# hangxu0304/DeepReduce

Measured on NVIDIA H100. Metric: ResNet-50 images/sec (whole job, device-timed, max over ranks), higher is better.
Workload: dtype bf16

## Files before the change

deepreduce_b200/models/resnet.py:

```python
from __future__ import annotations

import torch.nn as nn
import torch.nn.functional as F

from .fused_bn import bn_add_relu, bn_bn_add_relu, bn_relu, bn_relu_maxpool


class _BasicCifar(nn.Module):
    def __init__(self, inp, out, stride):
        super().__init__()
        self.conv1 = nn.Conv2d(inp, out, 3, stride, 1, bias=False)
        self.bn1 = nn.BatchNorm2d(out)
        self.conv2 = nn.Conv2d(out, out, 3, 1, 1, bias=False)
        self.bn2 = nn.BatchNorm2d(out)
        self.pad = None
        if stride != 1 or inp != out:
            self.pad = (out - inp, stride)

    def forward(self, x):
        y = F.relu(self.bn1(self.conv1(x)))
        y = self.bn2(self.conv2(y))
        if self.pad is not None:
            extra, s = self.pad
            x = F.pad(x[:, :, ::s, ::s], (0, 0, 0, 0, extra // 2, extra - extra // 2))
        return F.relu(x + y)


class ResNetCifar(nn.Module):
    def __init__(self, n: int = 3, num_classes: int = 10):
        super().__init__()
        self.conv1 = nn.Conv2d(3, 16, 3, 1, 1, bias=False)
        self.bn1 = nn.BatchNorm2d(16)
        layers, inp = [], 16
        for out, stride in ((16, 1), (32, 2), (64, 2)):
            for i in range(n):
                layers.append(_BasicCifar(inp, out, stride if i == 0 else 1))
                inp = out
        self.layers = nn.Sequential(*layers)
        self.fc = nn.Linear(64, num_classes)

    def forward(self, x):
        x = F.relu(self.bn1(self.conv1(x)))
        x = self.layers(x)
        x = F.adaptive_avg_pool2d(x, 1).flatten(1)
        return self.fc(x)


def resnet20(num_classes: int = 10) -> ResNetCifar:
    return ResNetCifar(3, num_classes)


class _Bottleneck(nn.Module):
    expansion = 4

    def __init__(self, inp, width, stride, downsample):
        super().__init__()
        out = width * self.expansion
        self.conv1 = nn.Conv2d(inp, width, 1, bias=False)
        self.bn1 = nn.BatchNorm2d(width)
        self.conv2 = nn.Conv2d(width, width, 3, stride, 1, bias=False)
        self.bn2 = nn.BatchNorm2d(width)
        self.conv3 = nn.Conv2d(width, out, 1, bias=False)
        self.bn3 = nn.BatchNorm2d(out)
        self.downsample = None
        if downsample:
            self.downsample = nn.Sequential(nn.Conv2d(inp, out, 1, stride, bias=False), nn.BatchNorm2d(out))

    def forward(self, x, skip=None, fork=False):
        skip = x if skip is None else skip
        xd = None if self.downsample is None else self.downsample[0](skip)
        y = bn_relu(self.conv1(x), self.bn1)
        y = bn_relu(self.conv2(y), self.bn2)
        y = self.conv3(y)
        if xd is None:
            return bn_add_relu(y, self.bn3, skip, fork=fork)
        o = bn_bn_add_relu(y, self.bn3, xd, self.downsample[1])
        return (o, None) if fork else o


class ResNet(nn.Module):
    def __init__(self, blocks=(3, 4, 6, 3), num_classes: int = 1000):
        super().__init__()
        self.conv1 = nn.Conv2d(3, 64, 7, 2, 3, bias=False)
        self.bn1 = nn.BatchNorm2d(64)
        self.maxpool = nn.MaxPool2d(3, 2, 1)
        stages, inp = [], 64
        for i, (n, width) in enumerate(zip(blocks, (64, 128, 256, 512))):
            for j in range(n):
                stride = 2 if (j == 0 and i > 0) else 1
                stages.append(_Bottleneck(inp, width, stride, downsample=(j == 0)))
                inp = width * 4
        self.layers = nn.Sequential(*stages)
        self.fc = nn.Linear(inp, num_classes)
        for m in self.modules():
            if isinstance(m, nn.Conv2d):
                nn.init.kaiming_normal_(m.weight, mode="fan_out", nonlinearity="relu")

    def forward(self, x):
        x, skip = bn_relu_maxpool(self.conv1(x), self.bn1, self.maxpool), None
        for blk in self.layers:
            x, skip = blk(x, skip, fork=True)
        x = F.adaptive_avg_pool2d(x, 1).flatten(1)
        return self.fc(x)


def resnet50(num_classes: int = 1000) -> ResNet:
    return ResNet((3, 4, 6, 3), num_classes)
```

deepreduce_b200/ops/csrc/bn.cu:

```cuda
#include <cuda_bf16.h>

#include <algorithm>

#include "common.cuh"
#include "ops.h"

namespace dr {

namespace {

constexpr int kVec = 8;
constexpr int kApplyThreads = 256;
constexpr int kReduceThreads = 128;

struct ChanParams {
  float m[kVec], inv[kVec], w[kVec], b[kVec];
};

__device__ __forceinline__ void load8(const float* __restrict__ p, float* d) {
  const float4 a = __ldg(reinterpret_cast<const float4*>(p));
  const float4 b = __ldg(reinterpret_cast<const float4*>(p) + 1);
  d[0] = a.x; d[1] = a.y; d[2] = a.z; d[3] = a.w;
  d[4] = b.x; d[5] = b.y; d[6] = b.z; d[7] = b.w;
}

__device__ __forceinline__ void load_params(const BnParams& p, int c, ChanParams& o) {
  load8(p.mean + c, o.m);
  load8(p.invstd + c, o.inv);
  load8(p.weight + c, o.w);
  load8(p.bias + c, o.b);
}

__device__ __forceinline__ float bn_elem(float x, float m, float inv, float w, float b) {
  return __fmaf_rn(__fmul_rn(w, __fsub_rn(x, m)), inv, b);
}

__device__ __forceinline__ __nv_bfloat16 relu_bf16(__nv_bfloat16 v) {
  return __bfloat162float(v) <= 0.f ? __float2bfloat16_rn(0.f) : v;
}

__device__ __forceinline__ uint4 add_bf16x8(const uint4& a, const uint4& b) {
  uint4 s;
  const __nv_bfloat16* ha = reinterpret_cast<const __nv_bfloat16*>(&a);
  const __nv_bfloat16* hb = reinterpret_cast<const __nv_bfloat16*>(&b);
  __nv_bfloat16* hs = reinterpret_cast<__nv_bfloat16*>(&s);
#pragma unroll
  for (int i = 0; i < kVec; ++i) hs[i] = __float2bfloat16_rn(__fadd_rn(__bfloat162float(ha[i]), __bfloat162float(hb[i])));
  return s;
}

template <int kMode>
__global__ void __launch_bounds__(kApplyThreads) bn_apply_kernel(const __nv_bfloat16* __restrict__ x, BnParams px,
                                                                 const __nv_bfloat16* __restrict__ z, BnParams pz,
                                                                 __nv_bfloat16* __restrict__ out,
                                                                 uint8_t* __restrict__ mask, int64_t rows, int C) {
  const int groups = C / kVec;
  const int rows_per_cta = blockDim.x / groups;
  const int rsub = threadIdx.x / groups;
  if (rsub >= rows_per_cta) return;
  const int c = (threadIdx.x % groups) * kVec;
  ChanParams a;
  load_params(px, c, a);
  ChanParams d;
  if (kMode == 2) load_params(pz, c, d);
  const int64_t step = (int64_t)gridDim.x * rows_per_cta;
#pragma unroll 2
  for (int64_t r = (int64_t)blockIdx.x * rows_per_cta + rsub; r < rows; r += step) {
    const int64_t off = r * C + c;
    const uint4 vx = *reinterpret_cast<const uint4*>(x + off);
    uint4 vz = make_uint4(0, 0, 0, 0);
    if (kMode != 0) vz = *reinterpret_cast<const uint4*>(z + off);
    const __nv_bfloat16* hx = reinterpret_cast<const __nv_bfloat16*>(&vx);
    const __nv_bfloat16* hz = reinterpret_cast<const __nv_bfloat16*>(&vz);
    uint4 vo;
    __nv_bfloat16* ho = reinterpret_cast<__nv_bfloat16*>(&vo);
    unsigned bits = 0;
#pragma unroll
    for (int i = 0; i < kVec; ++i) {
      __nv_bfloat16 y = __float2bfloat16_rn(bn_elem(__bfloat162float(hx[i]), a.m[i], a.inv[i], a.w[i], a.b[i]));
      if (kMode != 0) {
        const __nv_bfloat16 s = kMode == 1 ? hz[i]
                                           : __float2bfloat16_rn(bn_elem(__bfloat162float(hz[i]), d.m[i], d.inv[i], d.w[i], d.b[i]));
        y = __float2bfloat16_rn(__fadd_rn(__bfloat162float(y), __bfloat162float(s)));
      }
      ho[i] = relu_bf16(y);
      bits |= (__bfloat162float(ho[i]) <= 0.f ? 0u : 1u) << i;
    }
    *reinterpret_cast<uint4*>(out + off) = vo;
    mask[r * groups + c / kVec] = (uint8_t)bits;
  }
}


__global__ void __launch_bounds__(kApplyThreads) bn_apply_pool_kernel(const __nv_bfloat16* __restrict__ x, BnParams px,
                                                                      __nv_bfloat16* __restrict__ out,
                                                                      uint8_t* __restrict__ codes, int64_t orows,
                                                                      PoolGeom pg, int C) {
  const int groups = C / kVec;
  const int rows_per_cta = blockDim.x / groups;
  const int rsub = threadIdx.x / groups;
  if (rsub >= rows_per_cta) return;
  const int c = (threadIdx.x % groups) * kVec;
  ChanParams a;
  load_params(px, c, a);
  const int64_t step = (int64_t)gridDim.x * rows_per_cta;
  for (int64_t r = (int64_t)blockIdx.x * rows_per_cta + rsub; r < orows; r += step) {
    const int ow = (int)(r % pg.Wo);
    const int64_t t = r / pg.Wo;
    const int oh = (int)(t % pg.Ho);
    const int64_t n = t / pg.Ho;
    const int h0 = 2 * oh - 1, w0 = 2 * ow - 1;
    uint4 v[9];
#pragma unroll
    for (int k = 0; k < 9; ++k) {
      const int ih = h0 + k / 3, iw = w0 + k % 3;
      v[k] = ih >= 0 && ih < pg.H && iw >= 0 && iw < pg.W
                 ? *reinterpret_cast<const uint4*>(x + ((n * pg.H + ih) * pg.W + iw) * C + c)
                 : uint4{};
    }
    __nv_bfloat16 best[kVec];
    unsigned slot[kVec];
#pragma unroll
    for (int i = 0; i < kVec; ++i) {
      best[i] = __float2bfloat16_rn(-INFINITY);
      slot[i] = 0;
    }
#pragma unroll
    for (int k = 0; k < 9; ++k) {
      const int ih = h0 + k / 3, iw = w0 + k % 3;
      if (ih < 0 || ih >= pg.H || iw < 0 || iw >= pg.W) continue;
      const __nv_bfloat16* hx = reinterpret_cast<const __nv_bfloat16*>(&v[k]);
#pragma unroll
      for (int i = 0; i < kVec; ++i) {
        const __nv_bfloat16 y = relu_bf16(__float2bfloat16_rn(bn_elem(__bfloat162float(hx[i]), a.m[i], a.inv[i], a.w[i], a.b[i])));
        const float fy = __bfloat162float(y);
        if (fy > __bfloat162float(best[i]) || isnan(fy)) {
          best[i] = y;
          slot[i] = k;
        }
      }
    }
    uint4 vo;
    __nv_bfloat16* ho = reinterpret_cast<__nv_bfloat16*>(&vo);
    uint2 vc;
    uint8_t* hc = reinterpret_cast<uint8_t*>(&vc);
#pragma unroll
    for (int i = 0; i < kVec; ++i) {
      ho[i] = best[i];
      hc[i] = (uint8_t)(slot[i] | (__bfloat162float(best[i]) <= 0.f ? 0u : 0x80u));
    }
    *reinterpret_cast<uint4*>(out + r * C + c) = vo;
    *reinterpret_cast<uint2*>(codes + r * C + c) = vc;
  }
}

struct PoolGather {
  uint4 g[4];
  uint2 code[4];
  int off;
  int nh, nw;
  int sh, sw;
};

__device__ __forceinline__ void pool_gather_codes(PoolGather& q, const uint8_t* __restrict__ codes, const PoolGeom& pg,
                                                  int row, int C, int c, bool valid) {
  const int w = row % pg.W, t = row / pg.W, h = t % pg.H, n = t / pg.H;
  const int ph = h >> 1, pw = w >> 1;
  q.nh = valid ? min((h + 1) / 2 + 1, pg.Ho) - ph : 0;
  q.nw = valid ? min((w + 1) / 2 + 1, pg.Wo) - pw : 0;
  q.sh = h - 2 * ph + 1;
  q.sw = w - 2 * pw + 1;
  q.off = ((n * pg.Ho + ph) * pg.Wo + pw) * C + c;
#pragma unroll
  for (int k = 0; k < 4; ++k) {
    const int a = k >> 1, b = k & 1;
    q.code[k] = a < q.nh && b < q.nw ? *reinterpret_cast<const uint2*>(codes + q.off + (a * pg.Wo + b) * C) : uint2{};
  }
}

template <bool kTwo>
__device__ __forceinline__ void pool_gather_grads(PoolGather& q, const __nv_bfloat16* __restrict__ gp,
                                                  const __nv_bfloat16* __restrict__ gp2, const PoolGeom& pg, int C) {
#pragma unroll
  for (int k = 0; k < 4; ++k) {
    const int a = k >> 1, b = k & 1;
    const bool in = a < q.nh && b < q.nw;
    const int off = q.off + (a * pg.Wo + b) * C;
    q.g[k] = in ? *reinterpret_cast<const uint4*>(gp + off) : uint4{};
    if (kTwo && in) q.g[k] = add_bf16x8(q.g[k], *reinterpret_cast<const uint4*>(gp2 + off));
  }
}

__device__ __forceinline__ void pool_gather_resolve(const PoolGather& q, uint4& g, unsigned& bits) {
  __nv_bfloat16* hg = reinterpret_cast<__nv_bfloat16*>(&g);
  const bool single = q.nh == 1 && q.nw == 1;
  bits = 0;
#pragma unroll
  for (int i = 0; i < kVec; ++i) {
    float s = 0.f;
    __nv_bfloat16 one = __float2bfloat16_rn(0.f);
    unsigned bit = 0;
#pragma unroll
    for (int k = 0; k < 4; ++k) {
      const int a = k >> 1, b = k & 1;
      const unsigned code = (reinterpret_cast<const uint8_t*>(&q.code[k]))[i];
      if (a < q.nh && b < q.nw && (int)(code & 0x7fu) == (q.sh - 2 * a) * 3 + (q.sw - 2 * b)) {
        const __nv_bfloat16 v = (reinterpret_cast<const __nv_bfloat16*>(&q.g[k]))[i];
        s = __fadd_rn(s, __bfloat162float(v));
        one = v;
        bit = code >> 7;
      }
    }
    hg[i] = single ? one : __float2bfloat16_rn(s);
    bits |= bit << i;
  }
}

template <bool kTwo>
__global__ void __launch_bounds__(kApplyThreads) bn_pool_grad_kernel(const __nv_bfloat16* __restrict__ gp,
                                                                     const __nv_bfloat16* __restrict__ gp2,
                                                                     const uint8_t* __restrict__ codes,
                                                                     __nv_bfloat16* __restrict__ g, PoolGeom pg,
                                                                     int64_t rows, int C) {
  const int groups = C / kVec;
  const int rows_per_cta = blockDim.x / groups;
  const int rsub = threadIdx.x / groups;
  if (rsub >= rows_per_cta) return;
  const int c = (threadIdx.x % groups) * kVec;
  const int64_t step = (int64_t)gridDim.x * rows_per_cta;
#pragma unroll 2
  for (int64_t r = (int64_t)blockIdx.x * rows_per_cta + rsub; r < rows; r += step) {
    PoolGather q;
    pool_gather_codes(q, codes, pg, (int)r, C, c, true);
    pool_gather_grads<kTwo>(q, gp, gp2, pg, C);
    uint4 v;
    unsigned bits;
    pool_gather_resolve(q, v, bits);
    __nv_bfloat16* hv = reinterpret_cast<__nv_bfloat16*>(&v);
#pragma unroll
    for (int i = 0; i < kVec; ++i)
      if (!((bits >> i) & 1u)) hv[i] = __float2bfloat16_rn(0.f);
    *reinterpret_cast<uint4*>(g + r * C + c) = v;
  }
}

struct RowTree {
  int block_y, grid_y;
  __host__ __device__ int S() const { return block_y * grid_y; }
  __host__ __device__ int loops(int rows) const { return 1 + (rows - 1) / (S() * kLoads); }
  static constexpr int kLoads = 4;
};

constexpr int kStatsThreads = 256;

__device__ __forceinline__ void welford_update(float x, float inv, float valid, float& mean, float& m2n) {
  const float d0 = __fsub_rn(x, mean);
  mean = __fmaf_rn(d0, inv, mean);
  const float d1 = __fsub_rn(x, mean);
  m2n = __fmaf_rn(__fmul_rn(d0, d1), valid, m2n);
}

template <int kN, bool kFuseNew>
__device__ __forceinline__ void welford_merge(int& n, float* mean, float* m2n, int n_new, const float* mean_new,
                                              const float* m2n_new) {
  const float fn = (float)n, fn_new = (float)n_new;
  const float factor = __frcp_rn((float)max(1, n + n_new));
#pragma unroll
  for (int i = 0; i < kN; ++i) {
    const float d = __fsub_rn(mean[i], mean_new[i]);
    const float s = kFuseNew ? __fmaf_rn(mean_new[i], fn_new, __fmul_rn(mean[i], fn))
                             : __fmaf_rn(mean[i], fn, __fmul_rn(mean_new[i], fn_new));
    mean[i] = __fmul_rn(s, factor);
    const float u = __fmul_rn(__fmul_rn(__fmul_rn(d, d), fn_new), fn);
    m2n[i] = __fadd_rn(m2n[i], __fmaf_rn(u, factor, m2n_new[i]));
  }
  n += n_new;
}

template <int kN>
struct WelfordSlots {
  float* mean; float* m2n; int* count;
  __device__ WelfordSlots(float* sh, int slots)
      : mean(sh), m2n(sh + slots * kN), count(reinterpret_cast<int*>(sh + 2 * slots * kN)) {}
  __device__ void put(int s, int n, const float* m, const float* q) const {
#pragma unroll
    for (int i = 0; i < kN; ++i) { mean[s * kN + i] = m[i]; m2n[s * kN + i] = q[i]; }
    count[s] = n;
  }
  template <bool kFuseNew>
  __device__ void merge_from(int s, int& n, float* m, float* q) const {
    float mn[kN], qn[kN];
#pragma unroll
    for (int i = 0; i < kN; ++i) { mn[i] = mean[s * kN + i]; qn[i] = m2n[s * kN + i]; }
    welford_merge<kN, kFuseNew>(n, m, q, count[s], mn, qn);
  }
  static size_t bytes(int slots) { return (size_t)slots * (2 * kN * sizeof(float) + sizeof(int)); }
};

template <int kN>
__device__ __forceinline__ void welford_tree_over_y(const WelfordSlots<kN>& sl, bool part, int y, int block_y, int base,
                                                    int stride, int& n, float* mean, float* m2n) {
  for (int off = block_y / 2; off > 0; off >>= 1) {
    if (part && y < 2 * off) sl.put(base + y * stride, n, mean, m2n);
    __syncthreads();
    if (part && y < off) sl.template merge_from<false>(base + (y + off) * stride, n, mean, m2n);
    __syncthreads();
  }
}

struct StatsOut {
  float* mean; float* invstd; float* running_mean; float* running_var;
  float* st_mean; float* st_m2n; int* st_count;
  float momentum, bessel, eps;
};

__device__ __forceinline__ void stats_store(const StatsOut& o, int c, int n, float mean, float m2n) {
  const float var = __fdiv_rn(m2n, (float)n);
  const float keep = __fsub_rn(1.f, o.momentum);
  o.mean[c] = mean;
  o.invstd[c] = rsqrtf(__fadd_rn(var, o.eps));
  o.running_mean[c] = __fmaf_rn(mean, o.momentum, __fmul_rn(o.running_mean[c], keep));
  o.running_var[c] = __fmaf_rn(__fmul_rn(var, o.bessel), o.momentum, __fmul_rn(o.running_var[c], keep));
}

__global__ void __launch_bounds__(kStatsThreads) bn_stats_kernel(const __nv_bfloat16* __restrict__ x, StatsOut o,
                                                                 RowTree t, int rows, int C) {
  constexpr int L = RowTree::kLoads;
  constexpr int kAhead = 4;
  extern __shared__ float sh[];
  const int gpc = blockDim.x / (L * t.block_y);
  const int g = threadIdx.x % gpc, j = (threadIdx.x / gpc) % L, y = threadIdx.x / (gpc * L);
  const int group = blockIdx.x * gpc + g;
  const bool live = group * kVec < C;
  const int c = live ? group * kVec : 0;
  const int S = t.S();
  const int n_loops = t.loops(rows);
  const int r0 = blockIdx.y * t.block_y + y + j * S;
  const int rstep = L * S;
  float mean[kVec], m2n[kVec];
#pragma unroll
  for (int i = 0; i < kVec; ++i) mean[i] = m2n[i] = 0.f;
  int n = 0;
  auto load = [&](uint4* b, int i0) {
#pragma unroll
    for (int u = 0; u < kAhead; ++u) {
      const int r = r0 + (i0 + u) * rstep;
      b[u] = live && i0 + u < n_loops && r < rows ? *reinterpret_cast<const uint4*>(x + (size_t)r * C + c) : uint4{};
    }
  };
  uint4 cur[kAhead];
  load(cur, 0);
  for (int i0 = 0; i0 < n_loops; i0 += kAhead) {
    uint4 nxt[kAhead];
    load(nxt, i0 + kAhead);
#pragma unroll
    for (int u = 0; u < kAhead; ++u) {
      const int i = i0 + u;
      if (i >= n_loops) break;
      const bool valid = r0 + i * rstep < rows;
      const float inv = valid ? __frcp_rn((float)(i + 1)) : 0.f;
      const float fv = valid ? 1.f : 0.f;
      n += valid;
      const __nv_bfloat16* hx = reinterpret_cast<const __nv_bfloat16*>(&cur[u]);
#pragma unroll
      for (int k = 0; k < kVec; ++k) welford_update(__bfloat162float(hx[k]), inv, fv, mean[k], m2n[k]);
    }
#pragma unroll
    for (int u = 0; u < kAhead; ++u) cur[u] = nxt[u];
  }
  const WelfordSlots<kVec> sl(sh, blockDim.x);
  sl.put(threadIdx.x, n, mean, m2n);
  __syncthreads();
  if (j == 0) {
#pragma unroll
    for (int a = 1; a < L; ++a) sl.merge_from<true>(threadIdx.x + a * gpc, n, mean, m2n);
  }
  __syncthreads();
  welford_tree_over_y<kVec>(sl, j == 0, y, t.block_y, g, gpc * L, n, mean, m2n);
  if (j != 0 || y != 0 || !live) return;
  if (t.grid_y == 1) {
#pragma unroll
    for (int i = 0; i < kVec; ++i) stats_store(o, c + i, n, mean[i], m2n[i]);
    return;
  }
#pragma unroll
  for (int i = 0; i < kVec; ++i) {
    o.st_mean[(size_t)blockIdx.y * C + c + i] = mean[i];
    o.st_m2n[(size_t)blockIdx.y * C + c + i] = m2n[i];
  }
  if (group == 0) o.st_count[blockIdx.y] = n;
}

__global__ void bn_stats_finalize_kernel(StatsOut o, RowTree t, int C) {
  extern __shared__ float sh[];
  const int cols = blockDim.x / t.block_y;
  const int col = threadIdx.x % cols, y = threadIdx.x / cols;
  const int c = blockIdx.x * cols + col;
  int n = 0;
  float mean = 0.f, m2n = 0.f;
  if (c < C)
    for (int b = y; b < t.grid_y; b += t.block_y) {
      const float mb = o.st_mean[(size_t)b * C + c], qb = o.st_m2n[(size_t)b * C + c];
      welford_merge<1, false>(n, &mean, &m2n, o.st_count[b], &mb, &qb);
    }
  const WelfordSlots<1> sl(sh, blockDim.x);
  welford_tree_over_y<1>(sl, true, y, t.block_y, col, cols, n, &mean, &m2n);
  if (y == 0 && c < C) stats_store(o, c, n, mean, m2n);
}


template <int kN>
__device__ __forceinline__ void tree_over_y(float* v, float* sh, int y, int n, int col, int width) {
  for (int off = n / 2; off > 0; off >>= 1) {
#pragma unroll
    for (int i = 0; i < kN; ++i) sh[y * width + col + i] = v[i];
    __syncthreads();
    if (y < off) {
#pragma unroll
      for (int i = 0; i < kN; ++i) v[i] = __fadd_rn(v[i], sh[(y + off) * width + col + i]);
    }
    __syncthreads();
  }
}

struct BwdOut {
  float* sums;
  float* dw; float* db; float* dwz; float* dbz;
  float* staging;
};

__device__ __forceinline__ void bwd_store(const BwdOut& o, int k, int c, int C, float v, const float* invstd,
                                         const float* invstd_z) {
  o.sums[k * C + c] = v;
  if (k == 0) {
    o.db[c] = v;
    if (o.dbz) o.dbz[c] = v;
  } else if (k == 1) {
    o.dw[c] = __fmul_rn(v, invstd[c]);
  } else {
    o.dwz[c] = __fmul_rn(v, invstd_z[c]);
  }
}

__device__ __forceinline__ float masked(__nv_bfloat16 go, unsigned bit) { return bit ? __bfloat162float(go) : 0.f; }

template <int kMode, bool kTwo>
__global__ void __launch_bounds__(kReduceThreads) bn_bwd_reduce_kernel(const __nv_bfloat16* __restrict__ go,
                                                                       const __nv_bfloat16* __restrict__ go2,
                                                                       const uint8_t* __restrict__ mask,
                                                                       const __nv_bfloat16* __restrict__ x,
                                                                       const float* __restrict__ mean,
                                                                       const float* __restrict__ invstd,
                                                                       const __nv_bfloat16* __restrict__ z,
                                                                       const float* __restrict__ mean_z,
                                                                       const float* __restrict__ invstd_z,
                                                                       __nv_bfloat16* __restrict__ g_out, BwdOut o,
                                                                       RowTree t, int rows, int C) {
  constexpr int kSums = kMode == 2 ? 3 : 2;
  constexpr int L = RowTree::kLoads;
  extern __shared__ float sh[];
  const int gpc = blockDim.x / t.block_y;
  const int tg = threadIdx.x % gpc, y = threadIdx.x / gpc;
  const int group = blockIdx.x * gpc + tg;
  const bool live = group * kVec < C;
  const int c = live ? group * kVec : 0;
  const int S = t.S();
  float m[kVec], mz[kVec];
#pragma unroll
  for (int i = 0; i < kVec; ++i) {
    m[i] = mean[c + i];
    mz[i] = kMode == 2 ? mean_z[c + i] : 0.f;
  }
  float acc[kSums][L][kVec];
#pragma unroll
  for (int k = 0; k < kSums; ++k)
#pragma unroll
    for (int j = 0; j < L; ++j)
#pragma unroll
      for (int i = 0; i < kVec; ++i) acc[k][j][i] = 0.f;
  const int mgroups = C / kVec;
  int r = blockIdx.y * t.block_y + y;
  const int n_loops = t.loops(rows);
  constexpr bool kAhead = !(kTwo && kMode == 2);
  struct Batch {
    uint4 g[L], g2[L], x[L], z[L];
    unsigned m[L];
  };
  auto load = [&](Batch& b, int r0) {
#pragma unroll
    for (int j = 0; j < L; ++j) {
      const int rr = r0 + j * S;
      if (live && rr < rows) {
        const int off = rr * C + c;
        b.g[j] = *reinterpret_cast<const uint4*>(go + off);
        if (kTwo) b.g2[j] = *reinterpret_cast<const uint4*>(go2 + off);
        b.x[j] = *reinterpret_cast<const uint4*>(x + off);
        if (kMode == 2) b.z[j] = *reinterpret_cast<const uint4*>(z + off);
        b.m[j] = kMode == 3 ? 0u : mask[rr * mgroups + group];
      } else {
        b.g[j] = uint4{}; b.g2[j] = uint4{}; b.x[j] = uint4{}; b.z[j] = uint4{}; b.m[j] = 0;
      }
    }
  };
  Batch cur;
  if (kAhead) load(cur, r);
  for (int it = 0; it < n_loops; ++it) {
    if (!kAhead) load(cur, r);
    if (kTwo) {
#pragma unroll
      for (int j = 0; j < L; ++j) cur.g[j] = add_bf16x8(cur.g[j], cur.g2[j]);
    }
    Batch nxt;
    if (kAhead) load(nxt, r + L * S);
    const unsigned* mb = cur.m;
#pragma unroll
    for (int j = 0; j < L; ++j) {
      const __nv_bfloat16* hg = reinterpret_cast<const __nv_bfloat16*>(&cur.g[j]);
      const __nv_bfloat16* hx = reinterpret_cast<const __nv_bfloat16*>(&cur.x[j]);
      const __nv_bfloat16* hz = reinterpret_cast<const __nv_bfloat16*>(&cur.z[j]);
      uint4 vo;
      __nv_bfloat16* ho = reinterpret_cast<__nv_bfloat16*>(&vo);
#pragma unroll
      for (int i = 0; i < kVec; ++i) {
        const unsigned bit = (mb[j] >> i) & 1u;
        const float g = kMode == 3 ? __bfloat162float(hg[i]) : masked(hg[i], bit);
        if (kMode == 1) ho[i] = bit ? hg[i] : __float2bfloat16_rn(0.f);
        acc[0][j][i] = __fadd_rn(acc[0][j][i], g);
        acc[1][j][i] = __fmaf_rn(__fsub_rn(__bfloat162float(hx[i]), m[i]), g, acc[1][j][i]);
        if (kMode == 2) acc[2][j][i] = __fmaf_rn(__fsub_rn(__bfloat162float(hz[i]), mz[i]), g, acc[2][j][i]);
      }
      if (kMode == 1 && live && r + j * S < rows) *reinterpret_cast<uint4*>(g_out + (r + j * S) * C + c) = vo;
    }
    if (kAhead) cur = nxt;
    r += L * S;
  }
#pragma unroll
  for (int k = 0; k < kSums; ++k) {
#pragma unroll
    for (int i = 0; i < kVec; ++i)
#pragma unroll
      for (int j = 1; j < L; ++j) acc[k][0][i] = __fadd_rn(acc[k][0][i], acc[k][j][i]);
    tree_over_y<kVec>(acc[k][0], sh, y, t.block_y, tg * kVec, gpc * kVec);
  }
  if (y != 0 || !live) return;
#pragma unroll
  for (int k = 0; k < kSums; ++k)
#pragma unroll
    for (int i = 0; i < kVec; ++i) {
      if (t.grid_y > 1) o.staging[((size_t)k * t.grid_y + blockIdx.y) * C + c + i] = acc[k][0][i];
      else bwd_store(o, k, c + i, C, acc[k][0][i], invstd, invstd_z);
    }
}

__global__ void bn_bwd_finalize_kernel(BwdOut o, RowTree t, int n_sums, int C, const float* __restrict__ invstd,
                                       const float* __restrict__ invstd_z) {
  extern __shared__ float sh[];
  const int cols = blockDim.x / t.block_y;
  const int col = threadIdx.x % cols, y = threadIdx.x / cols;
  const int c = blockIdx.x * cols + col;
  for (int k = 0; k < n_sums; ++k) {
    float v = 0.f;
    if (c < C)
      for (int b = y; b < t.grid_y; b += t.block_y) v = __fadd_rn(v, o.staging[((size_t)k * t.grid_y + b) * C + c]);
    tree_over_y<1>(&v, sh, y, t.block_y, col, cols);
    if (y == 0 && c < C) bwd_store(o, k, c, C, v, invstd, invstd_z);
  }
}

struct ElemtChan {
  float m[kVec], f1[kVec], f2[kVec], sdy[kVec];
};

__device__ __forceinline__ void elemt_params(const float* mean, const float* invstd, const float* w, const float* sdy,
                                             const float* sxmu, float norm, int c, ElemtChan& p) {
  float inv[kVec], ww[kVec], sx[kVec];
  load8(mean + c, p.m);
  load8(invstd + c, inv);
  load8(w + c, ww);
  load8(sdy + c, p.sdy);
  load8(sxmu + c, sx);
#pragma unroll
  for (int i = 0; i < kVec; ++i) {
    p.f1[i] = __fmul_rn(__fmul_rn(__fmul_rn(inv[i], inv[i]), sx[i]), norm);
    p.f2[i] = __fmul_rn(ww[i], inv[i]);
  }
}

__device__ __forceinline__ __nv_bfloat16 elemt(float g, float x, const ElemtChan& p, int i, float norm) {
  const float a = __fmaf_rn(-p.sdy[i], norm, g);
  return __float2bfloat16_rn(__fmul_rn(__fmaf_rn(-p.f1[i], __fsub_rn(x, p.m[i]), a), p.f2[i]));
}

struct ElemtArgs {
  const float *mean, *invstd, *weight, *sums;
  const float *mean_z, *invstd_z, *weight_z;
};

template <int kMode, bool kTwo>
__global__ void __launch_bounds__(kApplyThreads) bn_bwd_elemt_kernel(const __nv_bfloat16* __restrict__ g_in,
                                                                     const __nv_bfloat16* __restrict__ g2_in,
                                                                     const uint8_t* __restrict__ mask,
                                                                     const __nv_bfloat16* __restrict__ x,
                                                                     const __nv_bfloat16* __restrict__ z, ElemtArgs a,
                                                                     __nv_bfloat16* __restrict__ dx,
                                                                     __nv_bfloat16* __restrict__ dz, float norm,
                                                                     int64_t rows, int C) {
  const int groups = C / kVec;
  const int rows_per_cta = blockDim.x / groups;
  const int rsub = threadIdx.x / groups;
  if (rsub >= rows_per_cta) return;
  const int c = (threadIdx.x % groups) * kVec;
  ElemtChan p;
  elemt_params(a.mean, a.invstd, a.weight, a.sums, a.sums + C, norm, c, p);
  ElemtChan q;
  if (kMode == 2) elemt_params(a.mean_z, a.invstd_z, a.weight_z, a.sums, a.sums + 2 * C, norm, c, q);
  const int64_t step = (int64_t)gridDim.x * rows_per_cta;
#pragma unroll 2
  for (int64_t r = (int64_t)blockIdx.x * rows_per_cta + rsub; r < rows; r += step) {
    const int64_t off = r * C + c;
    uint4 vg = *reinterpret_cast<const uint4*>(g_in + off);
    if (kTwo) vg = add_bf16x8(vg, *reinterpret_cast<const uint4*>(g2_in + off));
    const unsigned mb = kMode == 1 || kMode == 3 ? 0xffu : mask[r * groups + c / kVec];
    const uint4 vx = *reinterpret_cast<const uint4*>(x + off);
    uint4 vz = make_uint4(0, 0, 0, 0);
    if (kMode == 2) vz = *reinterpret_cast<const uint4*>(z + off);
    const __nv_bfloat16* hg = reinterpret_cast<const __nv_bfloat16*>(&vg);
    const __nv_bfloat16* hx = reinterpret_cast<const __nv_bfloat16*>(&vx);
    const __nv_bfloat16* hz = reinterpret_cast<const __nv_bfloat16*>(&vz);
    uint4 vo, vd;
    __nv_bfloat16* ho = reinterpret_cast<__nv_bfloat16*>(&vo);
    __nv_bfloat16* hd = reinterpret_cast<__nv_bfloat16*>(&vd);
#pragma unroll
    for (int i = 0; i < kVec; ++i) {
      const float g = masked(hg[i], (mb >> i) & 1u);
      ho[i] = elemt(g, __bfloat162float(hx[i]), p, i, norm);
      if (kMode == 2) hd[i] = elemt(g, __bfloat162float(hz[i]), q, i, norm);
    }
    *reinterpret_cast<uint4*>(dx + off) = vo;
    if (kMode == 2) *reinterpret_cast<uint4*>(dz + off) = vd;
  }
}

__global__ void bn_update_stats_kernel(const float* __restrict__ mean, float* __restrict__ var_invstd,
                                       float* __restrict__ running_mean, float* __restrict__ running_var, int C,
                                       float momentum, float bessel, float eps) {
  const int c = blockIdx.x * blockDim.x + threadIdx.x;
  if (c >= C) return;
  const float m = mean[c], v = var_invstd[c];
  const float unbiased_var = v * bessel;
  running_mean[c] = m * momentum + (1 - momentum) * running_mean[c];
  running_var[c] = unbiased_var * momentum + (1 - momentum) * running_var[c];
  var_invstd[c] = rsqrtf(v + eps);
}

template <typename K>
cudaError_t rows_grid(K kernel, int64_t rows, int C, int& grid, int& threads) {
  const int groups = C / kVec;
  const int rows_per_cta = groups >= kApplyThreads ? 1 : kApplyThreads / groups;
  threads = groups * rows_per_cta;
  int per_sm = 0;
  cudaError_t e = cudaOccupancyMaxActiveBlocksPerMultiprocessor(&per_sm, kernel, threads, 0);
  if (e != cudaSuccess) return e;
  int64_t g = (rows + rows_per_cta - 1) / rows_per_cta;
  const int64_t cap = (int64_t)(per_sm > 0 ? per_sm : 1) * sm_count();
  grid = (int)(g > cap ? cap : g);
  return cudaSuccess;
}

template <int kMode>
cudaError_t launch_apply(const void* x, const BnParams& px, const void* z, const BnParams& pz, void* out, void* mask,
                         int64_t rows, int C, cudaStream_t st) {
  if (rows == 0) return cudaSuccess;
  int grid = 0, threads = 0;
  cudaError_t e = rows_grid(bn_apply_kernel<kMode>, rows, C, grid, threads);
  if (e != cudaSuccess) return e;
  count_launch();
  bn_apply_kernel<kMode><<<grid, threads, 0, st>>>(reinterpret_cast<const __nv_bfloat16*>(x), px,
                                                   reinterpret_cast<const __nv_bfloat16*>(z), pz,
                                                   reinterpret_cast<__nv_bfloat16*>(out),
                                                   reinterpret_cast<uint8_t*>(mask), rows, C);
  return cudaGetLastError();
}

int last_pow2(unsigned n) {
  n |= n >> 1; n |= n >> 2; n |= n >> 4; n |= n >> 8; n |= n >> 16;
  return std::max<int>(1, (int)(n - (n >> 1)));
}

RowTree row_tree(int rows, int C) {
  const int block_x = std::min(last_pow2((unsigned)C), 32);
  const int block_y = std::min(last_pow2((unsigned)((rows + 15) / 16)), 512 / block_x);
  int grid_y = std::min((rows + block_y * 16 - 1) / (block_y * 16), 128);
  if (grid_y < 8) grid_y = 1;
  return {block_y, grid_y};
}

template <int kMode, bool kTwo>
cudaError_t launch_bwd_reduce(const BnBwd& b, const RowTree& t, const BwdOut& o, int rows, int C, cudaStream_t st) {
  const int groups = C / kVec;
  const int gpc = std::min(groups, std::max(1, kReduceThreads / t.block_y));
  const dim3 grid((groups + gpc - 1) / gpc, t.grid_y);
  const int threads = gpc * t.block_y;
  count_launch();
  bn_bwd_reduce_kernel<kMode, kTwo><<<grid, threads, threads * kVec * sizeof(float), st>>>(
      reinterpret_cast<const __nv_bfloat16*>(b.go), reinterpret_cast<const __nv_bfloat16*>(b.go2), b.mask,
      reinterpret_cast<const __nv_bfloat16*>(b.x), b.px.mean, b.px.invstd, reinterpret_cast<const __nv_bfloat16*>(b.z),
      b.pz.mean, b.pz.invstd, reinterpret_cast<__nv_bfloat16*>(b.g), o, t, rows, C);
  return cudaGetLastError();
}

template <int kMode, bool kTwo>
cudaError_t launch_bwd_elemt(const BnBwd& b, const ElemtArgs& a, int64_t rows, int C, cudaStream_t st) {
  int grid = 0, threads = 0;
  cudaError_t e = rows_grid(bn_bwd_elemt_kernel<kMode, kTwo>, rows, C, grid, threads);
  if (e != cudaSuccess) return e;
  const float norm = (float)(1.0 / (double)rows);
  count_launch();
  bn_bwd_elemt_kernel<kMode, kTwo><<<grid, threads, 0, st>>>(
      reinterpret_cast<const __nv_bfloat16*>(kMode == 1 || kMode == 3 ? b.g : b.go),
      reinterpret_cast<const __nv_bfloat16*>(b.go2), b.mask, reinterpret_cast<const __nv_bfloat16*>(b.x),
      reinterpret_cast<const __nv_bfloat16*>(b.z), a, reinterpret_cast<__nv_bfloat16*>(b.dx),
      reinterpret_cast<__nv_bfloat16*>(b.dz), norm, rows, C);
  return cudaGetLastError();
}

template <int kMode, bool kTwo>
cudaError_t launch_backward(const BnBwd& b, int64_t rows64, int C, cudaStream_t st) {
  const int rows = (int)rows64;
  const RowTree t = row_tree(rows, C);
  const BwdOut o{b.sums, b.dw, b.db, b.dwz, b.dbz, b.staging};
  cudaError_t e;
  if (kMode == 3) {
    int grid = 0, threads = 0;
    e = rows_grid(bn_pool_grad_kernel<kTwo>, rows64, C, grid, threads);
    if (e != cudaSuccess) return e;
    count_launch();
    bn_pool_grad_kernel<kTwo><<<grid, threads, 0, st>>>(reinterpret_cast<const __nv_bfloat16*>(b.go),
                                                        reinterpret_cast<const __nv_bfloat16*>(b.go2), b.mask,
                                                        reinterpret_cast<__nv_bfloat16*>(b.g), b.pool, rows64, C);
    e = cudaGetLastError();
    if (e != cudaSuccess) return e;
  }
  BnBwd bb = b;
  if (kMode == 3) bb.go = b.g;
  e = launch_bwd_reduce<kMode, kTwo && kMode != 3>(bb, t, o, rows, C, st);
  if (e != cudaSuccess) return e;
  if (t.grid_y > 1) {
    const int cols = std::max(1, 512 / t.block_y);
    const int threads = cols * t.block_y;
    count_launch();
    bn_bwd_finalize_kernel<<<(C + cols - 1) / cols, threads, threads * sizeof(float), st>>>(
        o, t, kMode == 2 ? 3 : 2, C, b.px.invstd, b.pz.invstd);
    e = cudaGetLastError();
    if (e != cudaSuccess) return e;
  }
  const ElemtArgs a{b.px.mean, b.px.invstd, b.px.weight, b.sums, b.pz.mean, b.pz.invstd, b.pz.weight};
  return launch_bwd_elemt<kMode, kTwo && kMode == 2>(b, a, rows64, C, st);
}

cudaError_t launch_stats(const BnStats& s, int rows, int C, cudaStream_t st) {
  const RowTree t = row_tree(rows, C);
  const int grid_y = t.grid_y;
  const StatsOut o{s.mean, s.invstd, s.running_mean, s.running_var,
                   s.staging, s.staging + (size_t)grid_y * C, reinterpret_cast<int*>(s.staging + 2 * (size_t)grid_y * C),
                   s.momentum, s.bessel, s.eps};
  const int groups = C / kVec;
  const int gpc = std::min(groups, std::max(1, kStatsThreads / (RowTree::kLoads * t.block_y)));
  const int threads = gpc * RowTree::kLoads * t.block_y;
  count_launch();
  bn_stats_kernel<<<dim3((groups + gpc - 1) / gpc, grid_y), threads, WelfordSlots<kVec>::bytes(threads), st>>>(
      reinterpret_cast<const __nv_bfloat16*>(s.x), o, t, rows, C);
  cudaError_t e = cudaGetLastError();
  if (e != cudaSuccess || grid_y == 1) return e;
  const int cols = std::max(1, 512 / t.block_y);
  const int fthreads = cols * t.block_y;
  count_launch();
  bn_stats_finalize_kernel<<<(C + cols - 1) / cols, fthreads, WelfordSlots<1>::bytes(fthreads), st>>>(o, t, C);
  return cudaGetLastError();
}

}

void bn_row_tree(int64_t rows, int C, int* block_y, int* grid_y) {
  const RowTree t = row_tree((int)rows, C);
  *block_y = t.block_y;
  *grid_y = t.grid_y;
}

cudaError_t launch_bn_backward(int mode, const BnBwd& b, int64_t rows, int C, cudaStream_t st) {
  if (rows == 0) return cudaSuccess;
  const bool two = b.go2 != nullptr;
  switch (mode) {
    case 0: return two ? cudaErrorInvalidValue : launch_backward<0, false>(b, rows, C, st);
    case 1: return two ? launch_backward<1, true>(b, rows, C, st) : launch_backward<1, false>(b, rows, C, st);
    case 2: return two ? launch_backward<2, true>(b, rows, C, st) : launch_backward<2, false>(b, rows, C, st);
    case 3: return two ? launch_backward<3, true>(b, rows, C, st) : launch_backward<3, false>(b, rows, C, st);
    default: return cudaErrorInvalidValue;
  }
}

cudaError_t launch_bn_stats(const BnStats& s, int64_t rows, int C, cudaStream_t st) {
  if (rows == 0) return cudaSuccess;
  return launch_stats(s, (int)rows, C, st);
}

cudaError_t launch_bn_update_stats(const float* mean, float* var_invstd, float* running_mean, float* running_var, int C,
                                   float momentum, float bessel, float eps, cudaStream_t st) {
  count_launch();
  bn_update_stats_kernel<<<(C + 255) / 256, 256, 0, st>>>(mean, var_invstd, running_mean, running_var, C, momentum,
                                                          bessel, eps);
  return cudaGetLastError();
}

cudaError_t launch_bn_apply(int mode, const void* x, const BnParams& px, const void* z, const BnParams& pz, void* out,
                            void* mask, int64_t rows, int C, cudaStream_t st) {
  switch (mode) {
    case 0: return launch_apply<0>(x, px, z, pz, out, mask, rows, C, st);
    case 1: return launch_apply<1>(x, px, z, pz, out, mask, rows, C, st);
    case 2: return launch_apply<2>(x, px, z, pz, out, mask, rows, C, st);
    default: return cudaErrorInvalidValue;
  }
}

cudaError_t launch_bn_apply_pool(const void* x, const BnParams& px, void* out, void* codes, int N, const PoolGeom& pg,
                                 int C, cudaStream_t st) {
  const int64_t orows = (int64_t)N * pg.Ho * pg.Wo;
  if (orows == 0) return cudaSuccess;
  int grid = 0, threads = 0;
  cudaError_t e = rows_grid(bn_apply_pool_kernel, orows, C, grid, threads);
  if (e != cudaSuccess) return e;
  count_launch();
  bn_apply_pool_kernel<<<grid, threads, 0, st>>>(reinterpret_cast<const __nv_bfloat16*>(x), px,
                                                 reinterpret_cast<__nv_bfloat16*>(out),
                                                 reinterpret_cast<uint8_t*>(codes), orows, pg, C);
  return cudaGetLastError();
}

}
```

Measured before the change: 6158.

## Tile fused BN-ReLU-maxpool forward and backward with shared-memory row reuse

Rewrites the stem BN+ReLU+maxpool forward kernel as a 2D-tiled kernel. A cp.async ring buffer stages input rows in shared memory, so each input pixel is normalized once and shared across overlapping 3x3 windows instead of being reloaded up to nine times. The pool-grad backward kernel is tiled the same way, walking output rows in bands and sharing neighbour gradients and codes through shared memory instead of gathering four per input pixel. The model also passes fork=True to the stem call, which changes the Python API expectation. It adds shared-memory use and __syncthreads, and relies on bn_relu_maxpool accepting the fork argument, which is not shown.

```diff
diff --git a/deepreduce_b200/models/resnet.py b/deepreduce_b200/models/resnet.py
--- a/deepreduce_b200/models/resnet.py
+++ b/deepreduce_b200/models/resnet.py
@@ -97,7 +97,7 @@
                 nn.init.kaiming_normal_(m.weight, mode="fan_out", nonlinearity="relu")
 
     def forward(self, x):
-        x, skip = bn_relu_maxpool(self.conv1(x), self.bn1, self.maxpool), None
+        x, skip = bn_relu_maxpool(self.conv1(x), self.bn1, self.maxpool, fork=True)
         for blk in self.layers:
             x, skip = blk(x, skip, fork=True)
         x = F.adaptive_avg_pool2d(x, 1).flatten(1)
diff --git a/deepreduce_b200/ops/csrc/bn.cu b/deepreduce_b200/ops/csrc/bn.cu
--- a/deepreduce_b200/ops/csrc/bn.cu
+++ b/deepreduce_b200/ops/csrc/bn.cu
@@ -91,105 +91,164 @@
   }
 }
 
-
-__global__ void __launch_bounds__(kApplyThreads) bn_apply_pool_kernel(const __nv_bfloat16* __restrict__ x, BnParams px,
-                                                                      __nv_bfloat16* __restrict__ out,
-                                                                      uint8_t* __restrict__ codes, int64_t orows,
-                                                                      PoolGeom pg, int C) {
-  const int groups = C / kVec;
-  const int rows_per_cta = blockDim.x / groups;
-  const int rsub = threadIdx.x / groups;
-  if (rsub >= rows_per_cta) return;
-  const int c = (threadIdx.x % groups) * kVec;
-  ChanParams a;
-  load_params(px, c, a);
-  const int64_t step = (int64_t)gridDim.x * rows_per_cta;
-  for (int64_t r = (int64_t)blockIdx.x * rows_per_cta + rsub; r < orows; r += step) {
-    const int ow = (int)(r % pg.Wo);
-    const int64_t t = r / pg.Wo;
-    const int oh = (int)(t % pg.Ho);
-    const int64_t n = t / pg.Ho;
-    const int h0 = 2 * oh - 1, w0 = 2 * ow - 1;
-    uint4 v[9];
-#pragma unroll
-    for (int k = 0; k < 9; ++k) {
-      const int ih = h0 + k / 3, iw = w0 + k % 3;
-      v[k] = ih >= 0 && ih < pg.H && iw >= 0 && iw < pg.W
-                 ? *reinterpret_cast<const uint4*>(x + ((n * pg.H + ih) * pg.W + iw) * C + c)
-                 : uint4{};
-    }
-    __nv_bfloat16 best[kVec];
-    unsigned slot[kVec];
-#pragma unroll
-    for (int i = 0; i < kVec; ++i) {
-      best[i] = __float2bfloat16_rn(-INFINITY);
-      slot[i] = 0;
-    }
-#pragma unroll
-    for (int k = 0; k < 9; ++k) {
-      const int ih = h0 + k / 3, iw = w0 + k % 3;
-      if (ih < 0 || ih >= pg.H || iw < 0 || iw >= pg.W) continue;
-      const __nv_bfloat16* hx = reinterpret_cast<const __nv_bfloat16*>(&v[k]);
-#pragma unroll
-      for (int i = 0; i < kVec; ++i) {
-        const __nv_bfloat16 y = relu_bf16(__float2bfloat16_rn(bn_elem(__bfloat162float(hx[i]), a.m[i], a.inv[i], a.w[i], a.b[i])));
-        const float fy = __bfloat162float(y);
-        if (fy > __bfloat162float(best[i]) || isnan(fy)) {
-          best[i] = y;
-          slot[i] = k;
-        }
-      }
-    }
-    uint4 vo;
-    __nv_bfloat16* ho = reinterpret_cast<__nv_bfloat16*>(&vo);
-    uint2 vc;
-    uint8_t* hc = reinterpret_cast<uint8_t*>(&vc);
-#pragma unroll
-    for (int i = 0; i < kVec; ++i) {
-      ho[i] = best[i];
-      hc[i] = (uint8_t)(slot[i] | (__bfloat162float(best[i]) <= 0.f ? 0u : 0x80u));
-    }
-    *reinterpret_cast<uint4*>(out + r * C + c) = vo;
-    *reinterpret_cast<uint2*>(codes + r * C + c) = vc;
-  }
+constexpr int kPoolThreads = 256;
+constexpr int kPoolSliceGroups = 32;
+constexpr int kPoolBand = 8;
+
+struct PoolTile {
+  int gs, slices;
+  int tile, tiles;
+  int band, bands;
+  int threads;
+  int64_t ctas;
+};
+
+struct PoolCta {
+  int64_t n;
+  int oh0, oh1;
+  int ow0;
+  int owl, gl, c;
+  bool group;
+};
+
+__device__ __forceinline__ PoolCta pool_cta(const PoolTile& t, const PoolGeom& pg, int C) {
+  PoolCta p;
+  int64_t b = blockIdx.x;
+  const int band = (int)(b % t.bands);
+  b /= t.bands;
+  const int tile = (int)(b % t.tiles);
+  b /= t.tiles;
+  const int slice = (int)(b % t.slices);
+  p.n = b / t.slices;
+  p.oh0 = band * t.band;
+  p.oh1 = min(p.oh0 + t.band, pg.Ho);
+  p.ow0 = tile * t.tile;
+  p.owl = threadIdx.x / t.gs;
+  p.gl = threadIdx.x % t.gs;
+  const int g = slice * t.gs + p.gl;
+  p.c = g * kVec;
+  p.group = g < C / kVec;
+  return p;
+}
+
+__device__ __forceinline__ uint4 bn_relu8(const uint4& vx, const ChanParams& a) {
+  uint4 vy;
+  const __nv_bfloat16* hx = reinterpret_cast<const __nv_bfloat16*>(&vx);
+  __nv_bfloat16* hy = reinterpret_cast<__nv_bfloat16*>(&vy);
+#pragma unroll
+  for (int i = 0; i < kVec; ++i)
+    hy[i] = relu_bf16(__float2bfloat16_rn(bn_elem(__bfloat162float(hx[i]), a.m[i], a.inv[i], a.w[i], a.b[i])));
+  return vy;
+}
+
+struct Win8 {
+  uint4 v;
+  uint2 s;
+};
+
+__device__ __forceinline__ Win8 win_init() {
+  const unsigned ninf2 = 0xff80ff80u;
+  return {make_uint4(ninf2, ninf2, ninf2, ninf2), make_uint2(0u, 0u)};
+}
+
+__device__ __forceinline__ void win_take(Win8& w, const uint4& v, const uint2& s) {
+  const unsigned* pv = &v.x;
+  unsigned* pw = &w.v.x;
+  unsigned m[4];
+#pragma unroll
+  for (int k = 0; k < 4; ++k) {
+    const __nv_bfloat162 a = *reinterpret_cast<const __nv_bfloat162*>(&pv[k]);
+    const __nv_bfloat162 b = *reinterpret_cast<const __nv_bfloat162*>(&pw[k]);
+    m[k] = __hgt2_mask(a, b) | __hneu2_mask(a, a);
+    pw[k] = (pv[k] & m[k]) | (pw[k] & ~m[k]);
+  }
+  const unsigned b0 = __byte_perm(m[0], m[1], 0x6420), b1 = __byte_perm(m[2], m[3], 0x6420);
+  w.s.x = (s.x & b0) | (w.s.x & ~b0);
+  w.s.y = (s.y & b1) | (w.s.y & ~b1);
+}
+
+constexpr unsigned kByte = 0x01010101u;
+
+__device__ __forceinline__ uint2 slot2(unsigned s) { return make_uint2(s, s); }
+
+constexpr int kPoolRing = 5;
+
+__device__ __forceinline__ void pool_fetch_row(uint4* slot, const __nv_bfloat16* __restrict__ xn, const PoolGeom& pg,
+                                               const PoolCta& p, const PoolTile& t, int C, int ih) {
+  const int ow = p.ow0 + p.owl - 1;
+  const __nv_bfloat16* row = xn + (int64_t)ih * pg.W * C;
+  if (p.group && p.owl > 0 && ow < pg.Wo) cp_async_16(slot + threadIdx.x, row + (int64_t)(2 * ow) * C);
+  if (p.group && ow >= 0 && 2 * ow + 1 < pg.W) cp_async_16(slot + t.threads + threadIdx.x, row + (int64_t)(2 * ow + 1) * C);
+}
+
+__device__ __forceinline__ Win8 pool_hscan(uint4* slot, const ChanParams& a, const PoolGeom& pg, const PoolCta& p,
+                                           const PoolTile& t) {
+  const int ow = p.ow0 + p.owl - 1;
+  const uint4 mid = bn_relu8(slot[threadIdx.x], a);
+  const uint4 right = bn_relu8(slot[t.threads + threadIdx.x], a);
+  slot[t.threads + threadIdx.x] = right;
+  __syncthreads();
+  Win8 w = win_init();
+  if (ow > 0) win_take(w, slot[t.threads + threadIdx.x - t.gs], slot2(0u));
+  win_take(w, mid, slot2(kByte));
+  if (2 * ow + 1 < pg.W) win_take(w, right, slot2(2 * kByte));
+  return w;
+}
+
+__global__ void __launch_bounds__(kPoolThreads, 3) bn_apply_pool_kernel(const __nv_bfloat16* __restrict__ x,
+                                                                        BnParams px, __nv_bfloat16* __restrict__ out,
+                                                                        uint8_t* __restrict__ codes, PoolGeom pg,
+                                                                        PoolTile t, int C) {
+  extern __shared__ uint4 pool_smem[];
+  const PoolCta p = pool_cta(t, pg, C);
+  const int ow = p.ow0 + p.owl - 1;
+  const bool out_thread = p.group && p.owl > 0 && ow < pg.Wo;
+  const __nv_bfloat16* xn = x + p.n * pg.H * pg.W * C + p.c;
+  const int r0 = max(2 * p.oh0 - 1, 0), rows = min(2 * p.oh1 - 1, pg.H - 1) - r0 + 1;
+  const int slot_elems = 2 * t.threads;
+#pragma unroll
+  for (int i = 0; i < kPoolRing - 1; ++i) {
+    if (i < rows) pool_fetch_row(pool_smem + i * slot_elems, xn, pg, p, t, C, r0 + i);
+    cp_async_commit();
+  }
+  ChanParams a{};
+  if (p.group) load_params(px, p.c, a);
+  Win8 up = win_init(), mid = win_init();
+  for (int i = 0; i < rows; ++i) {
+    cp_async_wait<kPoolRing - 2>();
+    const Win8 h = pool_hscan(pool_smem + (i % kPoolRing) * slot_elems, a, pg, p, t);
+    if (i + kPoolRing - 1 < rows)
+      pool_fetch_row(pool_smem + ((i + kPoolRing - 1) % kPoolRing) * slot_elems, xn, pg, p, t, C, r0 + i + kPoolRing - 1);
+    cp_async_commit();
+    if (!out_thread) continue;
+    const int ih = r0 + i;
+    if (!(ih & 1)) mid = h;
+    if ((ih & 1) ? ih > 2 * p.oh0 : ih == pg.H - 1) {
+      const int oh = ih >> 1;
+      Win8 w = win_init();
+      if (oh > 0) win_take(w, up.v, up.s);
+      win_take(w, mid.v, make_uint2(mid.s.x + 3 * kByte, mid.s.y + 3 * kByte));
+      if (ih & 1) win_take(w, h.v, make_uint2(h.s.x + 6 * kByte, h.s.y + 6 * kByte));
+      const __nv_bfloat16* hw = reinterpret_cast<const __nv_bfloat16*>(&w.v);
+      uint2 vc = w.s;
+      uint8_t* hc = reinterpret_cast<uint8_t*>(&vc);
+#pragma unroll
+      for (int k = 0; k < kVec; ++k) hc[k] |= __bfloat162float(hw[k]) <= 0.f ? 0u : 0x80u;
+      const int64_t off = ((p.n * pg.Ho + oh) * pg.Wo + ow) * C + p.c;
+      *reinterpret_cast<uint4*>(out + off) = w.v;
+      *reinterpret_cast<uint2*>(codes + off) = vc;
+    }
+    if (ih & 1) up = h;
+  }
+  cp_async_wait<0>();
 }
 
 struct PoolGather {
   uint4 g[4];
   uint2 code[4];
-  int off;
   int nh, nw;
   int sh, sw;
 };
-
-__device__ __forceinline__ void pool_gather_codes(PoolGather& q, const uint8_t* __restrict__ codes, const PoolGeom& pg,
-                                                  int row, int C, int c, bool valid) {
-  const int w = row % pg.W, t = row / pg.W, h = t % pg.H, n = t / pg.H;
-  const int ph = h >> 1, pw = w >> 1;
-  q.nh = valid ? min((h + 1) / 2 + 1, pg.Ho) - ph : 0;
-  q.nw = valid ? min((w + 1) / 2 + 1, pg.Wo) - pw : 0;
-  q.sh = h - 2 * ph + 1;
-  q.sw = w - 2 * pw + 1;
-  q.off = ((n * pg.Ho + ph) * pg.Wo + pw) * C + c;
-#pragma unroll
-  for (int k = 0; k < 4; ++k) {
-    const int a = k >> 1, b = k & 1;
-    q.code[k] = a < q.nh && b < q.nw ? *reinterpret_cast<const uint2*>(codes + q.off + (a * pg.Wo + b) * C) : uint2{};
-  }
-}
-
-template <bool kTwo>
-__device__ __forceinline__ void pool_gather_grads(PoolGather& q, const __nv_bfloat16* __restrict__ gp,
-                                                  const __nv_bfloat16* __restrict__ gp2, const PoolGeom& pg, int C) {
-#pragma unroll
-  for (int k = 0; k < 4; ++k) {
-    const int a = k >> 1, b = k & 1;
-    const bool in = a < q.nh && b < q.nw;
-    const int off = q.off + (a * pg.Wo + b) * C;
-    q.g[k] = in ? *reinterpret_cast<const uint4*>(gp + off) : uint4{};
-    if (kTwo && in) q.g[k] = add_bf16x8(q.g[k], *reinterpret_cast<const uint4*>(gp2 + off));
-  }
-}
 
 __device__ __forceinline__ void pool_gather_resolve(const PoolGather& q, uint4& g, unsigned& bits) {
   __nv_bfloat16* hg = reinterpret_cast<__nv_bfloat16*>(&g);
@@ -217,32 +276,83 @@
 }
 
 template <bool kTwo>
-__global__ void __launch_bounds__(kApplyThreads) bn_pool_grad_kernel(const __nv_bfloat16* __restrict__ gp,
-                                                                     const __nv_bfloat16* __restrict__ gp2,
-                                                                     const uint8_t* __restrict__ codes,
-                                                                     __nv_bfloat16* __restrict__ g, PoolGeom pg,
-                                                                     int64_t rows, int C) {
-  const int groups = C / kVec;
-  const int rows_per_cta = blockDim.x / groups;
-  const int rsub = threadIdx.x / groups;
-  if (rsub >= rows_per_cta) return;
-  const int c = (threadIdx.x % groups) * kVec;
-  const int64_t step = (int64_t)gridDim.x * rows_per_cta;
-#pragma unroll 2
-  for (int64_t r = (int64_t)blockIdx.x * rows_per_cta + rsub; r < rows; r += step) {
-    PoolGather q;
-    pool_gather_codes(q, codes, pg, (int)r, C, c, true);
-    pool_gather_grads<kTwo>(q, gp, gp2, pg, C);
-    uint4 v;
-    unsigned bits;
-    pool_gather_resolve(q, v, bits);
-    __nv_bfloat16* hv = reinterpret_cast<__nv_bfloat16*>(&v);
-#pragma unroll
-    for (int i = 0; i < kVec; ++i)
-      if (!((bits >> i) & 1u)) hv[i] = __float2bfloat16_rn(0.f);
-    *reinterpret_cast<uint4*>(g + r * C + c) = v;
-  }
-}
+__device__ __forceinline__ void pool_grad_row(const __nv_bfloat16* __restrict__ gp, const __nv_bfloat16* __restrict__ gp2,
+                                              const uint8_t* __restrict__ codes, const PoolGeom& pg, const PoolCta& p,
+                                              const PoolTile& t, int C, int oh, uint4* ws, uint2* cs, uint4& gv,
+                                              uint2& cv, uint4& gn, uint2& cn) {
+  const int ow = p.ow0 + p.owl;
+  const int64_t off = ((p.n * pg.Ho + oh) * pg.Wo + ow) * C + p.c;
+  gv = uint4{};
+  cv = uint2{};
+  if (p.group && ow < pg.Wo) {
+    gv = *reinterpret_cast<const uint4*>(gp + off);
+    cv = *reinterpret_cast<const uint2*>(codes + off);
+    if (kTwo) gv = add_bf16x8(gv, *reinterpret_cast<const uint4*>(gp2 + off));
+  }
+  ws[threadIdx.x] = gv;
+  cs[threadIdx.x] = cv;
+  __syncthreads();
+  gn = uint4{};
+  cn = uint2{};
+  if (p.owl < t.tile && ow + 1 < pg.Wo) {
+    gn = ws[threadIdx.x + t.gs];
+    cn = cs[threadIdx.x + t.gs];
+  }
+}
+
+template <bool kTwo>
+__global__ void __launch_bounds__(kPoolThreads, 3) bn_pool_grad_kernel(const __nv_bfloat16* __restrict__ gp,
+                                                                       const __nv_bfloat16* __restrict__ gp2,
+                                                                       const uint8_t* __restrict__ codes,
+                                                                       __nv_bfloat16* __restrict__ g, PoolGeom pg,
+                                                                       PoolTile t, int C) {
+  extern __shared__ uint4 pool_smem[];
+  const PoolCta p = pool_cta(t, pg, C);
+  const int ow = p.ow0 + p.owl;
+  const bool out_thread = p.group && p.owl < t.tile && ow < pg.Wo;
+  uint2* const cs = reinterpret_cast<uint2*>(pool_smem + 2 * t.threads);
+  __nv_bfloat16* gn = g + p.n * pg.H * pg.W * C + p.c;
+  PoolGather q;
+  pool_grad_row<kTwo>(gp, gp2, codes, pg, p, t, C, p.oh0, pool_smem, cs, q.g[0], q.code[0], q.g[1], q.code[1]);
+  int buf = 1;
+  for (int oh = p.oh0; oh < p.oh1; ++oh) {
+    const bool below = oh + 1 < pg.Ho;
+    if (below) {
+      pool_grad_row<kTwo>(gp, gp2, codes, pg, p, t, C, oh + 1, pool_smem + buf * t.threads, cs + buf * t.threads,
+                          q.g[2], q.code[2], q.g[3], q.code[3]);
+      buf ^= 1;
+    }
+    if (out_thread) {
+#pragma unroll
+      for (int dh = 0; dh < 2; ++dh) {
+        const int h = 2 * oh + dh;
+        if (h >= pg.H) break;
+        q.nh = dh == 1 && below ? 2 : 1;
+        q.sh = dh + 1;
+#pragma unroll
+        for (int dw = 0; dw < 2; ++dw) {
+          const int w = 2 * ow + dw;
+          if (w >= pg.W) break;
+          q.nw = dw == 1 && ow + 1 < pg.Wo ? 2 : 1;
+          q.sw = dw + 1;
+          uint4 v;
+          unsigned bits;
+          pool_gather_resolve(q, v, bits);
+          __nv_bfloat16* hv = reinterpret_cast<__nv_bfloat16*>(&v);
+#pragma unroll
+          for (int i = 0; i < kVec; ++i)
+            if (!((bits >> i) & 1u)) hv[i] = __float2bfloat16_rn(0.f);
+          *reinterpret_cast<uint4*>(gn + ((int64_t)h * pg.W + w) * C) = v;
+        }
+      }
+    }
+    q.g[0] = q.g[2];
+    q.code[0] = q.code[2];
+    q.g[1] = q.g[3];
+    q.code[1] = q.code[3];
+  }
+}
+
 
 struct RowTree {
   int block_y, grid_y;
@@ -667,6 +777,22 @@
   return cudaSuccess;
 }
 
+PoolTile pool_tile(const PoolGeom& pg, int N, int C) {
+  PoolTile t;
+  const int groups = C / kVec;
+  t.slices = (groups + kPoolSliceGroups - 1) / kPoolSliceGroups;
+  t.gs = (groups + t.slices - 1) / t.slices;
+  const int max_tile = kPoolThreads / t.gs - 1;
+  t.tiles = (pg.Wo + max_tile - 1) / max_tile;
+  t.tile = (pg.Wo + t.tiles - 1) / t.tiles;
+  t.bands = (pg.Ho + kPoolBand - 1) / kPoolBand;
+  t.band = (pg.Ho + t.bands - 1) / t.bands;
+  t.bands = (pg.Ho + t.band - 1) / t.band;
+  t.threads = (t.tile + 1) * t.gs;
+  t.ctas = (int64_t)N * t.bands * t.tiles * t.slices;
+  return t;
+}
+
 template <int kMode>
 cudaError_t launch_apply(const void* x, const BnParams& px, const void* z, const BnParams& pz, void* out, void* mask,
                          int64_t rows, int C, cudaStream_t st) {
@@ -731,13 +857,12 @@
   const BwdOut o{b.sums, b.dw, b.db, b.dwz, b.dbz, b.staging};
   cudaError_t e;
   if (kMode == 3) {
-    int grid = 0, threads = 0;
-    e = rows_grid(bn_pool_grad_kernel<kTwo>, rows64, C, grid, threads);
-    if (e != cudaSuccess) return e;
+    const PoolTile pt = pool_tile(b.pool, (int)(rows64 / ((int64_t)b.pool.H * b.pool.W)), C);
+    const size_t smem = 2 * (size_t)pt.threads * (sizeof(uint4) + sizeof(uint2));
     count_launch();
-    bn_pool_grad_kernel<kTwo><<<grid, threads, 0, st>>>(reinterpret_cast<const __nv_bfloat16*>(b.go),
-                                                        reinterpret_cast<const __nv_bfloat16*>(b.go2), b.mask,
-                                                        reinterpret_cast<__nv_bfloat16*>(b.g), b.pool, rows64, C);
+    bn_pool_grad_kernel<kTwo><<<(unsigned)pt.ctas, pt.threads, smem, st>>>(
+        reinterpret_cast<const __nv_bfloat16*>(b.go), reinterpret_cast<const __nv_bfloat16*>(b.go2), b.mask,
+        reinterpret_cast<__nv_bfloat16*>(b.g), b.pool, pt, C);
     e = cudaGetLastError();
     if (e != cudaSuccess) return e;
   }
@@ -824,15 +949,13 @@
 
 cudaError_t launch_bn_apply_pool(const void* x, const BnParams& px, void* out, void* codes, int N, const PoolGeom& pg,
                                  int C, cudaStream_t st) {
-  const int64_t orows = (int64_t)N * pg.Ho * pg.Wo;
-  if (orows == 0) return cudaSuccess;
-  int grid = 0, threads = 0;
-  cudaError_t e = rows_grid(bn_apply_pool_kernel, orows, C, grid, threads);
-  if (e != cudaSuccess) return e;
+  if ((int64_t)N * pg.Ho * pg.Wo == 0) return cudaSuccess;
+  const PoolTile pt = pool_tile(pg, N, C);
+  const size_t smem = (size_t)kPoolRing * 2 * pt.threads * sizeof(uint4);
   count_launch();
-  bn_apply_pool_kernel<<<grid, threads, 0, st>>>(reinterpret_cast<const __nv_bfloat16*>(x), px,
-                                                 reinterpret_cast<__nv_bfloat16*>(out),
-                                                 reinterpret_cast<uint8_t*>(codes), orows, pg, C);
+  bn_apply_pool_kernel<<<(unsigned)pt.ctas, pt.threads, smem, st>>>(reinterpret_cast<const __nv_bfloat16*>(x), px,
+                                                                    reinterpret_cast<__nv_bfloat16*>(out),
+                                                                    reinterpret_cast<uint8_t*>(codes), pg, pt, C);
   return cudaGetLastError();
 }
 
```

Result: faster. 6232 (median of 6 runs) (+1.2%).
